# delldu/TransMVSNet

Measured on AMD Instinct MI355X. Metric: depth maps/sec @ DTU 864x1152 N=5 (48/32/8 hyp); Abs depth L1 vs ref, higher is better.
Workload: dtype f32; 1 GPU; DTU 864x1152, N=5 views, cascade 48/32/8, B=1, hot path from FeatureNet outputs (FMT+pathway+stage glue+cost volume+CostRegNet+softmax/WTA); global_batch=1, parallelism=replica1, launch=hip_graph replay

## Files before the change

include/transmvs.h:

```cpp
#ifndef TRANSMVS_H_
#define TRANSMVS_H_

#include <stddef.h>

#ifdef __cplusplus
extern "C" {
#endif

#define TMVS_ABI_VERSION 11

#define TMVS_OK 0
#define TMVS_ERR_ARG (-1)
#define TMVS_ERR_SHAPE (-2)
#define TMVS_ERR_HIP (-3)

#define TMVS_MAX_VIEWS 16

int tmvs_abi_version(void);
const char* tmvs_status_string(int status);

int tmvs_bn_fold(const float* gamma, const float* beta, const float* mean, const float* var, int n, float eps,
                 float* alpha, float* shift);

int tmvs_stage_hypotheses(const float* depth_values, int n_values, const float* prev_depth, int prev_h, int prev_w,
                          int batch, int ndepth, float ratio, int full_h, int full_w, int stage_scale,
                          float* hyp_out, void* stream);

#define TMVS_WARP_PARTIAL 1
#define TMVS_WARP_ROT_PLAIN 2
#define TMVS_WARP_BWD_PLANES 4
#define TMVS_PW_NPARAMS 201
int tmvs_warp_corr(const float* ref_fea, const float* src_fea, const float* proj, const float* hyp,
                   const float* view_w_in, int vw_shift, int vw_offset, int vw_total, const float* pw_params,
                   int batch, int n_src, int channels, int ndepth, int height, int width, int flags,
                   float* sim_out, float* wsum_out, float* view_w_out, void* stream);

int tmvs_aggregate_finalize(float* sim_sum, const float* w_sum, int batch, int ndepth, int height, int width,
                            void* stream);

int tmvs_homo_warping(const float* src_fea, const float* proj, const float* hyp, int batch, int channels,
                      int ndepth, int height, int width, int flags, float* out, void* stream);

typedef struct {
  const float* w[11];
  const float* alpha[10];
  const float* shift[10];
  int base_ch;
} TmvsCostRegWeights;

size_t tmvs_costregnet_workspace(int batch, int depth, int height, int width, int base_ch);
int tmvs_costregnet(const float* x, int batch, int depth, int height, int width, const TmvsCostRegWeights* w,
                    void* workspace, size_t workspace_bytes, float* logits, void* stream);
int tmvs_costregnet_wta(const float* x, const float* hyp, int batch, int depth, int height, int width,
                        const TmvsCostRegWeights* w, void* workspace, size_t workspace_bytes, float clamp_lo,
                        float clamp_hi, float* prob, float* depth_out, float* depth_raw, float* conf, void* stream);

int tmvs_conv3d_bn_relu(const float* x, int batch, int cin, int d, int h, int w, const float* wpk, const float* alpha,
                        const float* shift, int cout, int stride, float* y, void* stream);
int tmvs_deconv3d_bn_relu_add(const float* x, int batch, int cin, int d, int h, int w, const float* wpk,
                              const float* alpha, const float* shift, int cout, const float* skip, float* y,
                              void* stream);

int tmvs_softmax_wta(const float* logits, const float* hyp, int batch, int ndepth, int height, int width,
                     float clamp_lo, float clamp_hi, float* prob, float* depth, float* depth_raw, float* conf,
                     void* stream);

#define TMVS_ENC_WQ 0
#define TMVS_ENC_BQ 1024
#define TMVS_ENC_WK 1056
#define TMVS_ENC_BK 2080
#define TMVS_ENC_WV 2112
#define TMVS_ENC_BV 3136
#define TMVS_ENC_WO 3168
#define TMVS_ENC_BO 4192
#define TMVS_ENC_W1 4224
#define TMVS_ENC_B1 6272
#define TMVS_ENC_W2T 6336
#define TMVS_ENC_B2 8384
#define TMVS_ENC_LN1G 8416
#define TMVS_ENC_LN1B 8448
#define TMVS_ENC_LN2G 8480
#define TMVS_ENC_LN2B 8512
#define TMVS_ENC_NPARAMS 8544
#define TMVS_KV_NFLOATS 160

int tmvs_fmt_embed(const float* feat, long feat_view_stride, const float* pe, int pe_h, int pe_w, int nv,
                   int channels, int height, int width, float* tokens, void* stream);
size_t tmvs_fmt_kv_workspace(int nv, int s_tokens);
int tmvs_fmt_kv(const float* source, int nv, int s_tokens, const float* enc_w, void* workspace,
                size_t workspace_bytes, float* kv, void* stream);
size_t tmvs_fmt_kv_grouped_workspace(int nv, int group_nv, int s_tokens);
int tmvs_fmt_kv_grouped(const float* source, int nv, int group_nv, int s_tokens, const float* enc_w, void* workspace,
                        size_t workspace_bytes, float* kv, void* stream);
int tmvs_fmt_apply(float* x, int nv, int l_tokens, const float* kv, long kv_view_stride, const float* enc_w,
                   void* stream);
int tmvs_fmt_apply_tiled(float* x, int nv, int l_tokens, const float* kv, long kv_view_stride, const float* enc_w,
                         int tiles_per_wave, void* stream);

int tmvs_fmt_pathway(const float* coarse, const float* lateral, long lat_view_stride, const float* w_reduce,
                     const float* w_smooth, int nv, int cc, int cf, int h, int w, float* out, void* stream);

size_t tmvs_fmt_forward_workspace(int nv, int l_tokens);
int tmvs_fmt_forward(const float* stage1, long view_stride, const float* pe, int pe_h, int pe_w, int nv, int height,
                     int width, const float* const* enc_w, void* workspace, size_t workspace_bytes, float* tokens,
                     void* stream);
size_t tmvs_fmt_forward_split_workspace(int nv, int l_tokens);
int tmvs_fmt_forward_split(const float* stage1, long view_stride, const float* pe, int pe_h, int pe_w, int nv,
                           int height, int width, const float* const* enc_w, void* workspace, size_t workspace_bytes,
                           float* tokens, void* stream, void* side_stream);

size_t tmvs_depth_stage_workspace(int ndepth, int height, int width, int base_ch);
int tmvs_depth_stage(const float* depth_values, int n_values, const float* prev_depth, int prev_h, int prev_w,
                     const float* feat, int n_views, int channels, int ndepth, float ratio, int full_h, int full_w,
                     int stage_scale, const float* proj, const float* pw_params, float* view_w, int vw_shift,
                     int warp_flags, const TmvsCostRegWeights* cr, void* workspace, size_t workspace_bytes, float clamp_lo,
                     float clamp_hi, float* hyp_out, float* prob_out, float* depth_out, float* depth_raw_out,
                     float* conf_out, void* stream);

#define TMVS_CONV_TRANSPOSED 1
#define TMVS_CONV_ACCUMULATE 2
int tmvs_conv3d_generic(const float* x, int batch, int cin, int d_in, int h_in, int w_in, const float* w, int cout,
                        int d_out, int h_out, int w_out, int stride, int flags, float* y, void* stream);

int tmvs_conv3d_mfma(const float* x, int batch, int cin, int d, int h, int w, const float* wpk, int cout, int stride,
                     int transposed, const float* skip, float* y, void* stream);

size_t tmvs_conv3d_wgrad_workspace(int batch, int d, int h, int w, int a_ch, int b_ch);
int tmvs_conv3d_wgrad(const float* direct, int a_ch, int batch, int pd, int ph, int pw, const float* gathered,
                      int b_ch, int gd, int gh, int gw, int stride, void* workspace, size_t workspace_bytes,
                      float* dw, void* stream);

size_t tmvs_warp_corr_backward_workspace(int n_src, int channels, int height, int width, int ndepth);
int tmvs_warp_corr_backward(const float* ref_fea, const float* src_fea, const float* proj, const float* hyp,
                            const float* dsim, int n_src, int channels, int ndepth, int height, int width, int flags,
                            void* workspace, size_t workspace_bytes, float* dref, float* dsrc, void* stream);

size_t tmvs_pixelwise_train_workspace(void);
int tmvs_pixelwise_train_forward(const float* sims, int n_views, int ndepth, int height, int width, const float* pwp,
                                 void* workspace, size_t workspace_bytes, float* stats, float* view_w, int* dstar,
                                 void* stream);
int tmvs_aggregate_train(const float* sims, const float* view_w, int n_views, int ndepth, int height, int width,
                         int vw_shift, float* sim, float* wsum, void* stream);
int tmvs_aggregate_train_backward(const float* dsim, const float* sims, const float* sim, const float* wsum,
                                  const float* view_w, int n_views, int ndepth, int height, int width, int vw_shift,
// ... 167 lines not shown
```

transmvsnet_amd/_lib.py:

```python
from __future__ import annotations

import ctypes
import os

_HERE = os.path.dirname(os.path.abspath(__file__))
LIB_PATH = os.environ.get("TMVS_LIB_PATH") or os.path.join(_HERE, "libtransmvs_hip.so")

P = ctypes.c_void_p
I = ctypes.c_int
L = ctypes.c_long
F = ctypes.c_float
S = ctypes.c_size_t
D = ctypes.c_double

SIGNATURES = {
    "tmvs_abi_version": (I, []),
    "tmvs_status_string": (ctypes.c_char_p, [I]),
    "tmvs_bn_fold": (I, [P, P, P, P, I, F, P, P]),
    "tmvs_stage_hypotheses": (I, [P, I, P, I, I, I, I, F, I, I, I, P, P]),
    "tmvs_warp_corr": (I, [P, P, P, P, P, I, I, I, P, I, I, I, I, I, I, I, P, P, P, P]),
    "tmvs_aggregate_finalize": (I, [P, P, I, I, I, I, P]),
    "tmvs_homo_warping": (I, [P, P, P, I, I, I, I, I, I, P, P]),
    "tmvs_costregnet_workspace": (S, [I, I, I, I, I]),
    "tmvs_costregnet": (I, [P, I, I, I, I, P, P, S, P, P]),
    "tmvs_costregnet_wta": (I, [P, P, I, I, I, I, P, P, S, F, F, P, P, P, P, P]),
    "tmvs_conv3d_bn_relu": (I, [P, I, I, I, I, I, P, P, P, I, I, P, P]),
    "tmvs_deconv3d_bn_relu_add": (I, [P, I, I, I, I, I, P, P, P, I, P, P, P]),
    "tmvs_softmax_wta": (I, [P, P, I, I, I, I, F, F, P, P, P, P, P]),
    "tmvs_fmt_embed": (I, [P, L, P, I, I, I, I, I, I, P, P]),
    "tmvs_fmt_kv_workspace": (S, [I, I]),
    "tmvs_fmt_kv": (I, [P, I, I, P, P, S, P, P]),
    "tmvs_fmt_apply": (I, [P, I, I, P, L, P, P]),
    "tmvs_fmt_apply_tiled": (I, [P, I, I, P, L, P, I, P]),
    "tmvs_fmt_pathway": (I, [P, P, L, P, P, I, I, I, I, I, P, P]),
    "tmvs_fmt_forward_workspace": (S, [I, I]),
    "tmvs_fmt_forward": (I, [P, L, P, I, I, I, I, I, P, P, S, P, P]),
    "tmvs_fmt_forward_split_workspace": (S, [I, I]),
    "tmvs_fmt_forward_split": (I, [P, L, P, I, I, I, I, I, P, P, S, P, P, P]),
    "tmvs_fmt_kv_grouped_workspace": (S, [I, I, I]),
    "tmvs_fmt_kv_grouped": (I, [P, I, I, I, P, P, S, P, P]),
    "tmvs_depth_stage_workspace": (S, [I, I, I, I]),
    "tmvs_depth_stage": (I, [P, I, P, I, I, P, I, I, I, F, I, I, I, P, P, P, I, I, P, P, S, F, F, P, P, P, P, P, P]),
    "tmvs_deform_conv2d_packed_floats": (S, [I]),
    "tmvs_deform_conv2d_pack": (I, [P, I, I, P]),
    "tmvs_deform_conv2d": (I, [P, P, P, P, P, P, I, I, I, I, I, I, P, P, P]),
    "tmvs_dcn_fused": (I, [P, P, P, P, P, P, P, I, I, I, I, I, I, P, P, P]),
    "tmvs_conv3x3_nhwc": (I, [P, P, P, P, P, I, I, I, I, I, I, P, P, P]),
    "tmvs_conv3x3_nhwc_acc": (I, [P, P, I, I, I, I, I, P, P]),
    "tmvs_fpn_merge": (I, [P, P, I, P, P, I, I, I, P, P]),
    "tmvs_conv2d_packed_floats": (S, [I, I, I]),
    "tmvs_conv2d_pack": (I, [P, I, I, I, P]),
    "tmvs_conv2d_bn_relu": (I, [P, I, I, I, I, P, I, I, I, P, P, I, P, P]),
    "tmvs_fusibile": (I, [P, P, I, I, I, I, I, F, P, P, P]),
    "tmvs_dynamic_fusion": (I, [P, I, I, I, I, P, I, P, P, P, F, I, I, P, P, P, P, P]),
    "tmvs_depth_postprocess": (I, [P, P, P, P, P, I, I, F, F, F, P, P, P, P, P]),
    "tmvs_resize_bilinear_u8": (I, [P, I, I, P, P, P, P, P, P, I, I, P, P]),
    "tmvs_resize_bilinear_f32": (I, [P, I, I, I, P, P, P, P, P, P, I, I, P, P]),
    "tmvs_entropy_loss_workspace": (S, [I, I, I]),
    "tmvs_entropy_loss": (I, [P, P, I, P, P, I, I, I, I, F, P, S, P, P, P, P, P]),
    "tmvs_depth_metrics_workspace": (S, [I]),
    "tmvs_depth_metrics": (I, [P, P, P, I, F, P, S, P, P]),
    "tmvs_warp_corr_backward_workspace": (S, [I, I, I, I, I]),
    "tmvs_warp_corr_backward": (I, [P, P, P, P, P, I, I, I, I, I, I, P, S, P, P, P]),
    "tmvs_pixelwise_train_workspace": (S, []),
    "tmvs_pixelwise_train_forward": (I, [P, I, I, I, I, P, P, S, P, P, P, P]),
    "tmvs_aggregate_train": (I, [P, P, I, I, I, I, I, P, P, P]),
    "tmvs_aggregate_train_backward": (I, [P, P, P, P, P, I, I, I, I, I, P, P, P]),
    "tmvs_pixelwise_train_backward": (I, [P, I, I, I, I, P, P, P, P, P, P, S, P, P, P]),
    "tmvs_upsample2_add_nhwc": (I, [P, P, I, I, I, I, P, P]),
    "tmvs_upsample2_backward_nhwc": (I, [P, I, I, I, I, P, P]),
    "tmvs_token_linear": (I, [P, L, I, I, P, P, I, P, I, P, P]),
    "tmvs_token_linear_res": (I, [P, L, I, I, P, P, I, P, P, P, P]),
    "tmvs_token_wgrad_workspace": (S, [L, I, I]),
    "tmvs_token_wgrad": (I, [P, I, P, I, L, P, S, P, P, I, P]),
    "tmvs_layer_norm_fwd": (I, [P, L, P, P, P, P]),
    "tmvs_layer_norm_bwd_workspace": (S, [L]),
    "tmvs_layer_norm_bwd": (I, [P, P, L, P, P, S, P, P, I, P]),
    "tmvs_linattn_fwd": (I, [P, L, L, P, L, P, P]),
    "tmvs_linattn_bwd_workspace": (S, [L, L]),
    "tmvs_linattn_bwd_q": (I, [P, P, L, L, P, L, P, S, P, P, P]),
    "tmvs_linattn_bwd_kv": (I, [P, P, L, L, P, P, P, P]),
    "tmvs_adam_step": (I, [P, P, P, P, L, D, D, D, D, D, I, P]),
    "tmvs_adam_step_dev": (I, [P, P, P, P, L, D, P, D, D, D, D, P, P, P]),
    "tmvs_conv3d_generic": (I, [P, I, I, I, I, I, P, I, I, I, I, I, I, P, P]),
    "tmvs_conv3d_mfma": (I, [P, I, I, I, I, I, P, I, I, I, P, P, P]),
    "tmvs_conv3d_wgrad_workspace": (S, [I, I, I, I, I, I]),
    "tmvs_conv3d_wgrad": (I, [P, I, I, I, I, I, P, I, I, I, I, I, P, S, P, P]),
    "tmvs_bn_train_workspace": (S, [L, I]),
    "tmvs_bn_stats": (I, [P, L, I, P, S, P, P, P]),
    "tmvs_bn_relu_train": (I, [P, L, I, P, P, P, P, F, P, P, P]),
    "tmvs_bn_relu_backward": (I, [P, P, L, I, P, P, P, P, F, P, S, P, P, P, P]),
    "tmvs_bn_train_workspace_grouped": (S, [I, L, I]),
    "tmvs_bn_stats_grouped": (I, [P, I, L, I, P, S, P, P, P]),
    "tmvs_bn_relu_train_grouped": (I, [P, I, L, I, P, P, P, P, F, P, P, P]),
    "tmvs_bn_relu_backward_grouped": (I, [P, P, I, L, I, P, P, P, P, F, P, S, P, P, P, P]),
    "tmvs_conv2d_generic": (I, [P, I, I, I, I, P, P, I, I, I, I, I, I, I, P, P]),
    "tmvs_conv2d_wgrad_workspace": (S, [I, I, I, I, I, I]),
    "tmvs_conv2d_wgrad": (I, [P, I, I, I, I, P, I, I, I, I, I, I, P, S, P, P]),
    "tmvs_colsum_workspace": (S, [L, I]),
    "tmvs_colsum": (I, [P, L, I, P, S, P, P]),
    "tmvs_dcn_forward_train": (I, [P, P, P, P, P, I, I, I, I, I, P, P, P, P]),
    "tmvs_dcn_backward_workspace": (S, [I, I, I, I]),
    "tmvs_dcn_backward": (I, [P, P, P, P, I, I, I, I, I, P, S, P, P, P, P]),
    "tmvs_dcn_backward_set": (I, [P, P, P, P, I, I, I, I, I, P, S, P, P, P, P, P]),
    "tmvs_nearest_up2_backward_nhwc": (I, [P, I, I, I, I, I, P, P]),
    "tmvs_softmax_backward": (I, [P, P, I, I, I, I, P, P]),
    "tmvs_dtu_cell_keys": (I, [P, L, P, P, P]),
    "tmvs_dtu_gather_points": (I, [P, P, P, L, P, P]),
    "tmvs_dtu_grid_table_bytes": (S, [L]),
    "tmvs_dtu_grid_table": (I, [P, P, L, L, P, S, P]),
# ... 52 lines not shown
```

transmvsnet_amd/csrc/costreg.hip:

```cpp
#include "common.h"

namespace tmvs {

typedef float floatx4 __attribute__((ext_vector_type(4)));

template <int N>
struct VecN;
template <>
struct VecN<4> {
  float v[4];
  __device__ __forceinline__ void load(const float* p) {
    const float4 t = *reinterpret_cast<const float4*>(p);
    v[0] = t.x;
    v[1] = t.y;
    v[2] = t.z;
    v[3] = t.w;
  }
  __device__ __forceinline__ void zero() { v[0] = v[1] = v[2] = v[3] = 0.f; }
};
template <>
struct VecN<2> {
  float v[2];
  __device__ __forceinline__ void load(const float* p) {
    const float2 t = *reinterpret_cast<const float2*>(p);
    v[0] = t.x;
    v[1] = t.y;
  }
  __device__ __forceinline__ void zero() { v[0] = v[1] = 0.f; }
};

struct Buf {
  __amdgpu_buffer_rsrc_t r;
  __device__ __forceinline__ Buf(const float* base, uint32_t nbytes)
      : r(__builtin_amdgcn_make_buffer_rsrc(const_cast<float*>(base), (short)0, (int)nbytes, 0x00020000)) {}
  static constexpr int kOOB = (int)0x80000000u;
  __device__ __forceinline__ float4 ld4(int voff, int soff = 0) const {
    const auto v = __builtin_amdgcn_raw_buffer_load_b128(r, voff, soff, 0);
    return make_float4(__uint_as_float(v[0]), __uint_as_float(v[1]), __uint_as_float(v[2]), __uint_as_float(v[3]));
  }
  __device__ __forceinline__ float2 ld2(int voff, int soff = 0) const {
    const auto v = __builtin_amdgcn_raw_buffer_load_b64(r, voff, soff, 0);
    return make_float2(__uint_as_float(v[0]), __uint_as_float(v[1]));
  }
};
template <int N>
__device__ __forceinline__ void buf_load(VecN<N>& d, const Buf& b, int voff, int soff = 0);
template <>
__device__ __forceinline__ void buf_load<4>(VecN<4>& d, const Buf& b, int voff, int soff) {
  const float4 t = b.ld4(voff, soff);
  d.v[0] = t.x, d.v[1] = t.y, d.v[2] = t.z, d.v[3] = t.w;
}
template <>
__device__ __forceinline__ void buf_load<2>(VecN<2>& d, const Buf& b, int voff, int soff) {
  const float2 t = b.ld2(voff, soff);
  d.v[0] = t.x, d.v[1] = t.y;
}

struct Geo {
  int Di, Hi, Wi;
  int Do, Ho, Wo;
  float lo;
};

__device__ __forceinline__ float act(float v, float lo) { return v > lo ? v : lo; }

constexpr int kLdsWavesPerEu = 3;
template <int CIN, int COUT, int S, int TD, int TH, int MBB, int WS = 1, bool KDSKIP = false, bool TAPOUT = false>
__global__ __launch_bounds__(256) __attribute__((amdgpu_waves_per_eu(kLdsWavesPerEu, kLdsWavesPerEu))) void conv3d_lds_kernel(const float* __restrict__ x, const float* __restrict__ wpk,
                                                         const float* __restrict__ alpha,
                                                         const float* __restrict__ shift, float* __restrict__ y,
                                                         Geo g) {
  constexpr int CK = CIN < 16 ? CIN : 16;
  constexpr int PL = CK / 4;
  constexpr int MB = (COUT + 15) / 16;
  constexpr int MG = MB / MBB;
  static_assert(WS == 1 || WS == 2 || WS == 4, "WS");
  static_assert(MBB % WS == 0 && (TD * TH * WS) % 4 == 0, "wave split");
  constexpr int NBW = TD * TH * WS / 4, MBW = MBB / WS;
  constexpr int LW = 15 * S + 3, LH = (TH - 1) * S + 3, LD = (TD - 1) * S + 3;
  constexpr bool SWZ = (CK == 16);
  constexpr int VST = SWZ ? 16 : CK + 4;
  constexpr int NVOX = LD * LH * LW;
  static_assert(MB % MBB == 0, "tile");
  static_assert(!TAPOUT || (TD == 1 && !KDSKIP), "TAPOUT: one output slice per workgroup, its own kd skip");
  __shared__ __attribute__((aligned(16))) float tile[(TAPOUT ? CIN / CK : 1) * NVOX * VST];

  const int nws = (g.Wo + 15) / 16, nhs = (g.Ho + TH - 1) / TH, nds = (g.Do + TD - 1) / TD;
  int t = xcd_remap(blockIdx.x, gridDim.x);
  const int mg = t % MG;
  t /= MG;
  const int ws = t % nws;
  t /= nws;
  const int hs = t % nhs;
  t /= nhs;
  const int ds = t % nds;
  const int n = t / nds;
  const int ow0 = ws * 16, oh0 = hs * TH, od0 = ds * TD;
  const int iw0 = ow0 * S - 1, ih0 = oh0 * S - 1, id0 = od0 * S - 1;
  const int lane = threadIdx.x & 63, wv = threadIdx.x >> 6;
  const int col = lane & 15, kgrp = lane >> 4;
  const int rg = __builtin_amdgcn_readfirstlane(wv / WS), bg = __builtin_amdgcn_readfirstlane(wv % WS);
  const int mb0 = mg * MBB + bg * MBW;
  const size_t in_n = (size_t)n * g.Di * g.Hi * g.Wi;

  floatx4 acc[NBW][MBW];
#pragma unroll
  for (int r = 0; r < NBW; ++r)
#pragma unroll
    for (int m = 0; m < MBW; ++m) acc[r][m] = floatx4{0.f, 0.f, 0.f, 0.f};

  constexpr int NCH = CIN / CK, NLD = (NVOX * PL + 255) / 256;
  const Buf xb(x + in_n * CIN, (uint32_t)g.Di * g.Hi * g.Wi * CIN * 4);
  const Buf wb(wpk, 27u * COUT * CIN * 4);
  float4 pf[NLD];
  auto fetch_to = [&](int ch, float4(&dst)[NLD]) {
#pragma unroll
    for (int k = 0; k < NLD; ++k) {
      const int idx = threadIdx.x + 256 * k;
      const int vox = idx / PL, q = idx - vox * PL;
      const int lw = vox % LW, rest = vox / LW, lh = rest % LH, ld = rest / LH;
      const int iw = iw0 + lw, ih = ih0 + lh, id = id0 + ld;
// ... 954 lines not shown
    bool ok[NBW];
#pragma unroll
    for (int r = 0; r < NBW; ++r) {
      const int rr = wv * NBW + r;
      const int md = c.md0 + rr / THI, mh = c.mh0 + rr % THI;
      ok[r] = md < g.Di && mh < g.Hi && ow < 2 * g.Wi;
      oo[r] = (out_n + ((size_t)(2 * md) * g.Ho + 2 * mh) * g.Wo + ow) * 8 + (lane & 1) * 4;
#pragma unroll
      for (int pdh = 0; pdh < 4; ++pdh)
        sk[r][pdh] = (ok[r] && skip) ? *reinterpret_cast<const float4*>(skip + oo[r] + (pdh >> 1) * plane + (pdh & 1) * row)
                           : make_float4(0.f, 0.f, 0.f, 0.f);
    }
    floatx4 acc[NBW][4];
#pragma unroll
    for (int r = 0; r < NBW; ++r)
#pragma unroll
      for (int q = 0; q < 4; ++q) acc[r][q] = floatx4{0.f, 0.f, 0.f, 0.f};
#pragma unroll
    for (int pdh = 0; pdh < 4; ++pdh) {
      const int pd = pdh >> 1, ph = pdh & 1;
#pragma unroll
      for (int td = 0; td < 1 + pd; ++td)
#pragma unroll
        for (int th = 0; th < 1 + ph; ++th) {
          const int kd = pd ? (td ? 2 : 0) : 1, od_off = (pd && !td) ? 1 : 0;
          const int kh = ph ? (th ? 2 : 0) : 1, oh_off = (ph && !th) ? 1 : 0;
          const int tap_base = kd * 9 + kh * 3;
          VecN<PL> a1, a2;
          wfrag(tap_base + (hi ? 2 : 1), a1);
          if (hi)
            wfrag(tap_base + 0, a2);
          else
            a2.zero();
#pragma unroll
          for (int r = 0; r < NBW; ++r) {
            const int rr = wv * NBW + r;
            const int mdl = rr / THI, mhl = rr - mdl * THI;
            const int lv = ((mdl + od_off) * LH + mhl + oh_off) * LW + col;
            VecN<PL> b1, b2;
            b1.load(cur + lv * VST + 4 * (kgrp ^ ((lv >> 1) & 3)));
            b2.load(cur + (lv + 1) * VST + 4 * (kgrp ^ (((lv + 1) >> 1) & 3)));
#pragma unroll
            for (int j = 0; j < PL; ++j)
              acc[r][pdh] = __builtin_amdgcn_mfma_f32_16x16x4f32(a1.v[j], b1.v[j], acc[r][pdh], 0, 0, 0);
#pragma unroll
            for (int j = 0; j < PL; ++j)
              acc[r][pdh] = __builtin_amdgcn_mfma_f32_16x16x4f32(a2.v[j], b2.v[j], acc[r][pdh], 0, 0, 0);
          }
          __builtin_amdgcn_sched_barrier(0);
        }
    }
#pragma unroll
    for (int r = 0; r < NBW; ++r)
#pragma unroll
      for (int pdh = 0; pdh < 4; ++pdh) {
        const floatx4 a = acc[r][pdh];
        *reinterpret_cast<float4*>(eb + (2 * col + (kgrp >> 1)) * 8 + cq) =
            make_float4(act(fmaf(a[0], al.x, sh.x), g.lo), act(fmaf(a[1], al.y, sh.y), g.lo), act(fmaf(a[2], al.z, sh.z), g.lo),
                        act(fmaf(a[3], al.w, sh.w), g.lo));
        __builtin_amdgcn_wave_barrier();
        const float4 v = *reinterpret_cast<const float4*>(eb + lane * 4);
        __builtin_amdgcn_wave_barrier();
        const float4 sv = sk[r][pdh];
        if (ok[r])
          *reinterpret_cast<float4*>(y + oo[r] + (pdh >> 1) * plane + (pdh & 1) * row) =
              make_float4(sv.x + v.x, sv.y + v.y, sv.z + v.z, sv.w + v.w);
      }
    if (tn < t_hi) commit(tile[(it + 1) & 1]);
    __syncthreads();
  }
}

template <int TDI, int THI>
static int launch_deconv_c8(const float* x, const float* w, const float* al, const float* sh, const float* skip,
                            float* y, int B, const Geo& g, hipStream_t st) {
  const long ntiles = (long)B * ((g.Di + TDI - 1) / TDI) * ((g.Hi + THI - 1) / THI) * ((g.Wi + 15) / 16);
  const long grid = persistent_grid(deconv3d_c8_kernel<TDI, THI>, ntiles);
  hipLaunchKernelGGL((deconv3d_c8_kernel<TDI, THI>), dim3((unsigned)grid), dim3(256), 0, st, x, w, al, sh, skip, y, g,
                     (int)ntiles);
  TMVS_CHECK_LAUNCH();
  return TMVS_OK;
}

template <int CIN, int COUT, int TDI, int THI, int MBB>
static int launch_deconv(const float* x, const float* w, const float* al, const float* sh, const float* skip,
                         float* y, int B, const Geo& g, hipStream_t st) {
  constexpr int MG = ((COUT + 15) / 16) / MBB;
  const long nblk = (long)B * ((g.Di + TDI - 1) / TDI) * ((g.Hi + THI - 1) / THI) * ((g.Wi + 15) / 16) * MG;
  hipLaunchKernelGGL((deconv3d_lds_kernel<CIN, COUT, TDI, THI, MBB>), dim3((unsigned)nblk), dim3(256), 0, st, x, w,
                     al, sh, skip, y, g);
  TMVS_CHECK_LAUNCH();
  return TMVS_OK;
}

static int conv_dispatch(const float* x, int B, int cin, int d, int h, int w, const float* wpk, const float* al,
                         const float* sh, int cout, int stride, float* y, hipStream_t st, float lo = 0.f) {
  Geo g;
  g.lo = lo;
  g.Di = d;
  g.Hi = h;
  g.Wi = w;
  if (stride == 1) {
    g.Do = d;
    g.Ho = h;
    g.Wo = w;
  } else {
    g.Do = (d - 1) / 2 + 1;
    g.Ho = (h - 1) / 2 + 1;
    g.Wo = (w - 1) / 2 + 1;
  }
  if ((long long)d * h * w * cin * 4 >= (1LL << 31)) return TMVS_ERR_SHAPE;
  constexpr int kKdSkipMaxDo = 2;
  const bool kdskip = g.Do <= kKdSkipMaxDo;
  constexpr bool KD = true, TAPOUT = true;
  using Conv3Tile = LdsTile<2, 2, 2, 2>;
  using Conv4Tile = LdsTile<2, 2, 2, 2>;
  using Conv4TileKd = LdsTile<2, 4, 2, 1>;
  using Conv5Tile = LdsTile<1, 2, 4, 4>;
  using Conv6Tile = LdsTile<1, 2, 4, 4>;
  int (*launch)(const float*, const float*, const float*, const float*, float*, int, const Geo&, hipStream_t) = nullptr;
  if (stride == 1) {
    if (cin == 16 && cout == 16)
      launch = launch_conv_c16<2, 4>;
    else if (cin == 32 && cout == 32)
      launch = kdskip ? launch_conv<32, 32, 1, Conv4TileKd, KD> : launch_conv<32, 32, 1, Conv4Tile>;
    else if (cin == 64 && cout == 64)
      launch = kdskip ? launch_conv<64, 64, 1, Conv6Tile, KD> : launch_conv<64, 64, 1, Conv6Tile>;
  } else {
    if (cin == 8 && cout == 16)
      launch = launch_conv_s2c8_tile<2, 2>;
    else if (cin == 16 && cout == 32)
      launch = kdskip ? launch_conv<16, 32, 2, Conv3Tile, KD> : launch_conv<16, 32, 2, Conv3Tile>;
    else if (cin == 32 && cout == 64)
      launch = launch_conv<32, 64, 2, Conv5Tile, false, TAPOUT>;
  }
  return launch ? launch(x, wpk, al, sh, y, B, g, st) : TMVS_ERR_SHAPE;
}

static int deconv_dispatch(const float* x, int B, int cin, int d, int h, int w, const float* wpk, const float* al,
                           const float* sh, int cout, const float* skip, float* y, hipStream_t st, float lo = 0.f) {
  Geo g;
  g.lo = lo;
  g.Di = d;
  g.Hi = h;
  g.Wi = w;
  g.Do = 2 * d;
  g.Ho = 2 * h;
  g.Wo = 2 * w;
  const bool even = g.Di % 2 == 0;
  int (*launch)(const float*, const float*, const float*, const float*, const float*, float*, int, const Geo&,
                hipStream_t) = nullptr;
  if (cin == 64 && cout == 32)
    launch = even ? launch_deconv<64, 32, 2, 2, 1> : launch_deconv<64, 32, 1, 4, 1>;
  else if (cin == 32 && cout == 16)
    launch = even ? launch_deconv<32, 16, 2, 2, 1> : launch_deconv<32, 16, 1, 4, 1>;
  else if (cin == 16 && cout == 8)
    launch = even ? launch_deconv_c8<2, 2> : launch_deconv_c8<1, 4>;
  return launch ? launch(x, wpk, al, sh, skip, y, B, g, st) : TMVS_ERR_SHAPE;
}


}

using namespace tmvs;

extern "C" int tmvs_conv3d_bn_relu(const float* x, int batch, int cin, int d, int h, int w, const float* wpk,
                                   const float* alpha, const float* shift, int cout, int stride, float* y,
                                   void* stream) {
  if (!x || !wpk || !alpha || !shift || !y || batch <= 0 || d <= 0 || h <= 0 || w <= 0) return TMVS_ERR_ARG;
  if (stride != 1 && stride != 2) return TMVS_ERR_ARG;
  return conv_dispatch(x, batch, cin, d, h, w, wpk, alpha, shift, cout, stride, y, (hipStream_t)stream);
}

extern "C" int tmvs_deconv3d_bn_relu_add(const float* x, int batch, int cin, int d, int h, int w, const float* wpk,
                                         const float* alpha, const float* shift, int cout, const float* skip,
                                         float* y, void* stream) {
  if (!x || !wpk || !alpha || !shift || !skip || !y || batch <= 0 || d <= 0 || h <= 0 || w <= 0)
    return TMVS_ERR_ARG;
  return deconv_dispatch(x, batch, cin, d, h, w, wpk, alpha, shift, cout, skip, y, (hipStream_t)stream);
}

static int launch_prob(const float* x, float* y, int batch, int D, int H, int W, const float* wt, hipStream_t st) {
  constexpr int NR = 1;
  const dim3 grid((unsigned)(((W + kProbCols - 1) / kProbCols) * ((H + 4 * NR - 1) / (4 * NR)) * batch *
                             ((D + kDChunk - 1) / kDChunk)));
  hipLaunchKernelGGL(prob_kernel<NR>, grid, dim3(256), 0, st, x, y, D, H, W, wt);
  TMVS_CHECK_LAUNCH();
  return TMVS_OK;
}

__device__ float kUnitAlpha[64] = {1.f, 1.f, 1.f, 1.f, 1.f, 1.f, 1.f, 1.f, 1.f, 1.f, 1.f, 1.f, 1.f, 1.f, 1.f, 1.f,
                                   1.f, 1.f, 1.f, 1.f, 1.f, 1.f, 1.f, 1.f, 1.f, 1.f, 1.f, 1.f, 1.f, 1.f, 1.f, 1.f,
                                   1.f, 1.f, 1.f, 1.f, 1.f, 1.f, 1.f, 1.f, 1.f, 1.f, 1.f, 1.f, 1.f, 1.f, 1.f, 1.f,
                                   1.f, 1.f, 1.f, 1.f, 1.f, 1.f, 1.f, 1.f, 1.f, 1.f, 1.f, 1.f, 1.f, 1.f, 1.f, 1.f};
__device__ float kZeroShift[64];

extern "C" int tmvs_conv3d_mfma(const float* x, int batch, int cin, int d, int h, int w, const float* wpk, int cout,
                                int stride, int transposed, const float* skip, float* y, void* stream) {
  if (!x || !wpk || !y || batch <= 0 || d <= 0 || h <= 0 || w <= 0) return TMVS_ERR_ARG;
  if (transposed ? stride != 2 : (stride != 1 && stride != 2)) return TMVS_ERR_ARG;
  if (skip && !transposed) return TMVS_ERR_ARG;
  int dev = 0;
  if (hipGetDevice(&dev) != hipSuccess || dev < 0 || dev >= 64) return TMVS_ERR_HIP;
  static const float* unit[64][2];
  if (!unit[dev][0]) {
    void *a, *b;
    if (hipGetSymbolAddress(&a, HIP_SYMBOL(kUnitAlpha)) != hipSuccess ||
        hipGetSymbolAddress(&b, HIP_SYMBOL(kZeroShift)) != hipSuccess)
      return TMVS_ERR_HIP;
    unit[dev][1] = (const float*)b;
    unit[dev][0] = (const float*)a;
  }
  const float *al = unit[dev][0], *sh = unit[dev][1];
  const float lo = -__builtin_huge_valf();
  hipStream_t st = (hipStream_t)stream;
  if (!transposed && stride == 1 && cin == 1 && cout == 8) {
    if ((long long)d * h * w * 32 >= (1LL << 31)) return TMVS_ERR_SHAPE;
    const dim3 grid((unsigned)(((w + kProbCols - 1) / kProbCols) * ((h + 3) / 4) * batch * ((d + kDChunk - 1) / kDChunk)));
    hipLaunchKernelGGL(conv0_kernel, grid, dim3(256), 0, st, x, y, d, h, w, wpk, al, sh, lo);
    TMVS_CHECK_LAUNCH();
    return TMVS_OK;
  }
  if (!transposed && stride == 1 && cin == 8 && cout == 1) {
    if ((long long)d * h * w * 32 >= (1LL << 31)) return TMVS_ERR_SHAPE;
    return launch_prob(x, y, batch, d, h, w, wpk, st);
  }
  if (transposed) return deconv_dispatch(x, batch, cin, d, h, w, wpk, al, sh, cout, skip, y, st, lo);
  return conv_dispatch(x, batch, cin, d, h, w, wpk, al, sh, cout, stride, y, st, lo);
}

static size_t align_up(size_t v) { return (v + 255) & ~(size_t)255; }

extern "C" size_t tmvs_costregnet_workspace(int batch, int depth, int height, int width, int base_ch) {
  const size_t v0 = (size_t)batch * depth * height * width;
  const size_t v1 = v0 / 8, v2 = v0 / 64, v3 = v0 / 512;
  const size_t c = (size_t)base_ch;
  size_t bytes = 0;
  bytes += align_up(v0 * c * 4);
  bytes += align_up(v1 * 2 * c * 4) * 2;
  bytes += align_up(v2 * 4 * c * 4) * 2;
  bytes += align_up(v3 * 8 * c * 4) * 2;
  bytes += align_up(v2 * 4 * c * 4);
  bytes += align_up(v1 * 2 * c * 4);
  bytes += align_up(v0 * c * 4);
  return bytes;
}

static int costregnet_trunk(const float* x, int batch, int depth, int height, int width, const TmvsCostRegWeights* w,
                            void* workspace, size_t workspace_bytes, hipStream_t st, float** x11_out,
                            float** c0_out) {
  if (!x || !w || !workspace || batch <= 0) return TMVS_ERR_ARG;
  if (depth % 8 || height % 8 || width % 8) return TMVS_ERR_SHAPE;
  if (w->base_ch != 8) return TMVS_ERR_SHAPE;
  if ((long long)depth * height * width * 32 >= (1LL << 31)) return TMVS_ERR_SHAPE;
  for (int i = 0; i < 11; ++i)
    if (!w->w[i]) return TMVS_ERR_ARG;
  for (int i = 0; i < 10; ++i)
    if (!w->alpha[i] || !w->shift[i]) return TMVS_ERR_ARG;
  if (workspace_bytes < tmvs_costregnet_workspace(batch, depth, height, width, w->base_ch)) return TMVS_ERR_ARG;
  const int c = w->base_ch;
  const size_t v0 = (size_t)batch * depth * height * width;
  const size_t v1 = v0 / 8, v2 = v0 / 64, v3 = v0 / 512;
// ... 93 lines not shown
```

transmvsnet_amd/ops.py:

```python
from __future__ import annotations

import ctypes

import numpy as np
import torch

from . import _lib

_lib_h = _lib.load


_TIMER = None


def set_timer(timer):
    global _TIMER
    _TIMER = timer


class _Span:
    __slots__ = ("tok",)

    def __init__(self, name):
        self.tok = _TIMER.begin(name) if _TIMER is not None else None
# ... 185 lines not shown


def costregnet(x, weights: "_lib.CostRegWeights", keepalive=None):
    _dev(x, "x")
    b, d, h, w = x.shape
    nbytes = _lib_h().tmvs_costregnet_workspace(b, d, h, w, weights.base_ch)
    ws = torch.empty(nbytes // 4 + 64, device=x.device)
    out = torch.empty_like(x)
    with _Span("tmvs_costregnet"):
        _lib.check(_lib_h().tmvs_costregnet(_ptr(x), b, d, h, w, ctypes.byref(weights), _ptr(ws), ws.numel() * 4,
                                            _ptr(out), _stream()), "tmvs_costregnet")
    return out


def costregnet_wta(x, weights: "_lib.CostRegWeights", hyp, clamp=(425.0, 935.0)):
    _dev(x, "x")
    _dev(hyp, "hyp")
    b, d, h, w = x.shape
    if tuple(hyp.shape) != (b, d, h, w):
        raise ValueError(f"costregnet_wta: hyp shape {tuple(hyp.shape)} != volume shape {(b, d, h, w)}")
    nbytes = _lib_h().tmvs_costregnet_workspace(b, d, h, w, weights.base_ch)
    ws = torch.empty(nbytes // 4 + 64, device=x.device)
    prob = torch.empty_like(x)
    depth = torch.empty(b, h, w, device=x.device)
    raw = torch.empty_like(depth)
    conf = torch.empty_like(depth)
    with _Span("tmvs_costregnet"):
        _lib.check(_lib_h().tmvs_costregnet_wta(_ptr(x), _ptr(hyp), b, d, h, w, ctypes.byref(weights), _ptr(ws),
                                                ws.numel() * 4, ctypes.c_float(clamp[0]), ctypes.c_float(clamp[1]),
                                                _ptr(prob), _ptr(depth), _ptr(raw), _ptr(conf), _stream()),
                   "tmvs_costregnet_wta")
    return prob, depth, raw, conf


def _layer_args(op, x, wpk, alpha, shift, cout):
    if x.dim() != 5:
        raise ValueError(f"{op}: x must be NDHWC [B, D, H, W, cin]")
    for name, t in (("x", x), ("wpk", wpk), ("alpha", alpha), ("shift", shift)):
        _layer_tensor(op, name, t, x.device)
    cin = x.shape[4]
    if wpk.numel() != 27 * cout * cin:
        raise ValueError(f"{op}: wpk must hold 27 * cout * cin = {27 * cout * cin} floats, not {wpk.numel()}")
    for name, t in (("alpha", alpha), ("shift", shift)):
        if t is not None and t.numel() < cout:
            raise ValueError(f"{op}: {name} must hold cout = {cout} floats, not {t.numel()}")


def _layer_tensor(op, name, t, device):
    if t is None:
        return
    if not t.is_cuda or t.device != device:
        raise ValueError(f"{op}: {name} must be a GPU tensor on x's device (the HIP path has no CPU fallback)")
    if t.dtype != torch.float32 or not t.is_contiguous():
        raise ValueError(f"{op}: {name} must be contiguous float32")


def _layer_like(op, name, t, shape, device):
    _layer_tensor(op, name, t, device)
    if t is not None and tuple(t.shape) != tuple(shape):
        raise ValueError(f"{op}: {name} must be a contiguous {list(shape)} tensor, not {list(t.shape)}")


def _layer_no_alias(op, skip, out):
    if skip is not None and out is not None and skip.data_ptr() == out.data_ptr():
        raise ValueError(f"{op}: out must not alias skip (the kernels read skip while they write out)")


def _conv_out_dhw(d, h, w, stride):
    return (d, h, w) if stride == 1 else ((d - 1) // 2 + 1, (h - 1) // 2 + 1, (w - 1) // 2 + 1)


def conv3d_bn_relu(x, wpk, alpha, shift, cout, stride, out=None):
    _layer_args("conv3d_bn_relu", x, wpk, alpha, shift, cout)
    b, d, h, w, cin = x.shape
    shape = (b, *_conv_out_dhw(d, h, w, stride), cout)
    _layer_like("conv3d_bn_relu", "out", out, shape, x.device)
    y = torch.empty(shape, device=x.device) if out is None else out
    with _Span("tmvs_conv3d_bn_relu"):
        _lib.check(_lib_h().tmvs_conv3d_bn_relu(_ptr(x), b, cin, d, h, w, _ptr(wpk), _ptr(alpha), _ptr(shift), cout,
                                                stride, _ptr(y), _stream()), "tmvs_conv3d_bn_relu")
    return y


def deconv3d_bn_relu_add(x, wpk, alpha, shift, cout, skip, out=None):
    _layer_args("deconv3d_bn_relu_add", x, wpk, alpha, shift, cout)
    b, d, h, w, cin = x.shape
    shape = (b, 2 * d, 2 * h, 2 * w, cout)
    if skip is None:
        raise ValueError("deconv3d_bn_relu_add: skip is required")
    _layer_like("deconv3d_bn_relu_add", "skip", skip, shape, x.device)
    _layer_like("deconv3d_bn_relu_add", "out", out, shape, x.device)
    _layer_no_alias("deconv3d_bn_relu_add", skip, out)
    y = torch.empty(shape, device=x.device) if out is None else out
    with _Span("tmvs_deconv3d_bn_relu_add"):
        _lib.check(_lib_h().tmvs_deconv3d_bn_relu_add(_ptr(x), b, cin, d, h, w, _ptr(wpk), _ptr(alpha), _ptr(shift),
                                                      cout, _ptr(skip), _ptr(y), _stream()), "tmvs_deconv3d_bn_relu_add")
    return y


def fmt_embed(feat_nchw, pe, out_tokens):
    nv, c, h, w = feat_nchw.shape
    with _Span("tmvs_fmt_embed"):
        _lib.check(_lib_h().tmvs_fmt_embed(_ptr(feat_nchw), c * h * w, _ptr(pe), pe.shape[1], pe.shape[2], nv, c, h, w,
                                           _ptr(out_tokens), _stream()), "tmvs_fmt_embed")
    return out_tokens


def fmt_kv(source_tokens, enc_w, out=None, group_nv=None):
    nv, s, _ = source_tokens.shape
    group_nv = nv if group_nv is None else int(group_nv)
    nbytes = _lib_h().tmvs_fmt_kv_grouped_workspace(nv, group_nv, s)
    ws = torch.empty(max(1, nbytes // 4), device=source_tokens.device)
    kv = out if out is not None else torch.empty(nv, _lib.KV_NFLOATS, device=source_tokens.device)
    with _Span("tmvs_fmt_kv"):
        _lib.check(_lib_h().tmvs_fmt_kv_grouped(_ptr(source_tokens), nv, group_nv, s, _ptr(enc_w), _ptr(ws),
                                                ws.numel() * 4, _ptr(kv), _stream()), "tmvs_fmt_kv_grouped")
    return kv


def fmt_apply(x_tokens, kv, enc_w, shared_kv=False, tiles_per_wave=0):
    nv, l, _ = x_tokens.shape
    with _Span("tmvs_fmt_apply"):
        _lib.check(_lib_h().tmvs_fmt_apply_tiled(_ptr(x_tokens), nv, l, _ptr(kv), 0 if shared_kv else _lib.KV_NFLOATS,
                                                 _ptr(enc_w), int(tiles_per_wave), _stream()), "tmvs_fmt_apply")
    return x_tokens


def fmt_pathway(coarse_nhwc, lateral_nchw, w_reduce, w_smooth, out=None):
    nv, h, w, cc = coarse_nhwc.shape
    cf = lateral_nchw.shape[1]
    if out is None:
        out = torch.empty(nv, 2 * h, 2 * w, cf, device=coarse_nhwc.device)
    elif tuple(out.shape) != (nv, 2 * h, 2 * w, cf) or not out.is_contiguous():
        raise ValueError(f"fmt_pathway: out must be a contiguous [{nv},{2 * h},{2 * w},{cf}] tensor")
    with _Span("tmvs_fmt_pathway"):
        _lib.check(_lib_h().tmvs_fmt_pathway(_ptr(coarse_nhwc), _ptr(lateral_nchw), cf * 4 * h * w, _ptr(w_reduce),
                                             _ptr(w_smooth), nv, cc, cf, h, w, _ptr(out), _stream()), "tmvs_fmt_pathway")
    return out


def fmt_forward(stage1_nchw, pe, enc_list, tokens=None, side_stream=None):
    _dev(stage1_nchw, "stage1")
    nv, c, h, w = stage1_nchw.shape
    tokens = torch.empty(nv, h * w, c, device=stage1_nchw.device) if tokens is None else tokens
    split = side_stream is not None and nv > 1
    lib = _lib_h()
    nbytes = lib.tmvs_fmt_forward_split_workspace(nv, h * w) if split else lib.tmvs_fmt_forward_workspace(nv, h * w)
    ws = torch.empty(nbytes // 4 + 64, device=stage1_nchw.device)
    ptrs = (ctypes.c_void_p * 8)(*[e.data_ptr() for e in enc_list])
    args = (_ptr(stage1_nchw), c * h * w, _ptr(pe), pe.shape[1], pe.shape[2], nv, h, w, ptrs, _ptr(ws), ws.numel() * 4,
            _ptr(tokens), _stream())
    with _Span("tmvs_fmt_forward"):
        if split:
            _lib.check(lib.tmvs_fmt_forward_split(*args, side_stream.cuda_stream), "tmvs_fmt_forward_split")
            if not torch.cuda.is_current_stream_capturing():
                ws.record_stream(side_stream)
                tokens.record_stream(side_stream)
        else:
            _lib.check(lib.tmvs_fmt_forward(*args), "tmvs_fmt_forward")
    return tokens


def depth_stage(depth_values, prev_depth, feat_nhwc, ndepth, ratio, full_hw, stage_scale, proj12, pw_params,
                view_w, vw_shift, cr_weights, clamp=(425.0, 935.0), rot_order="auto"):
    _dev(depth_values, "depth_values")
    _dev(prev_depth, "prev_depth")
    _dev(feat_nhwc, "feat")
    _dev(view_w, "view_w")
    n, h, w, c = feat_nhwc.shape
    dev = feat_nhwc.device
    hyp = torch.empty(1, ndepth, h, w, device=dev)
    prob = torch.empty_like(hyp)
    depth = torch.empty(1, h, w, device=dev)
    raw = torch.empty_like(depth)
    conf = torch.empty_like(depth)
    nbytes = _lib_h().tmvs_depth_stage_workspace(ndepth, h, w, cr_weights.base_ch)
    ws = torch.empty(nbytes // 4 + 64, device=dev)
    proj = np.ascontiguousarray(proj12, np.float32).reshape(n - 1, 12)
    pw = None if pw_params is None else np.ascontiguousarray(pw_params, np.float32)
# ... 881 lines not shown
```

Before: 302.3 depth_maps/s.

## Add persistent software-pipelined MFMA kernel for 32→16 transposed 3D conv

```diff
diff --git a/include/transmvs.h b/include/transmvs.h
--- a/include/transmvs.h
+++ b/include/transmvs.h
@@ -60,6 +60,12 @@
 int tmvs_deconv3d_bn_relu_add(const float* x, int batch, int cin, int d, int h, int w, const float* wpk,
                               const float* alpha, const float* shift, int cout, const float* skip, float* y,
                               void* stream);
+int tmvs_deconv3d_bn_relu_add_generic(const float* x, int batch, int cin, int d, int h, int w, const float* wpk,
+                                      const float* alpha, const float* shift, int cout, const float* skip, float* y,
+                                      void* stream);
+int tmvs_deconv3d_bn_relu_add_persistent(const float* x, int batch, int cin, int d, int h, int w, const float* wpk,
+                                         const float* alpha, const float* shift, int cout, const float* skip,
+                                         float* y, int max_workgroups, void* stream);
 
 int tmvs_softmax_wta(const float* logits, const float* hyp, int batch, int ndepth, int height, int width,
                      float clamp_lo, float clamp_hi, float* prob, float* depth, float* depth_raw, float* conf,
diff --git a/transmvsnet_amd/_lib.py b/transmvsnet_amd/_lib.py
--- a/transmvsnet_amd/_lib.py
+++ b/transmvsnet_amd/_lib.py
@@ -26,6 +26,8 @@
     "tmvs_costregnet_wta": (I, [P, P, I, I, I, I, P, P, S, F, F, P, P, P, P, P]),
     "tmvs_conv3d_bn_relu": (I, [P, I, I, I, I, I, P, P, P, I, I, P, P]),
     "tmvs_deconv3d_bn_relu_add": (I, [P, I, I, I, I, I, P, P, P, I, P, P, P]),
+    "tmvs_deconv3d_bn_relu_add_generic": (I, [P, I, I, I, I, I, P, P, P, I, P, P, P]),
+    "tmvs_deconv3d_bn_relu_add_persistent": (I, [P, I, I, I, I, I, P, P, P, I, P, P, I, P]),
     "tmvs_softmax_wta": (I, [P, P, I, I, I, I, F, F, P, P, P, P, P]),
     "tmvs_fmt_embed": (I, [P, L, P, I, I, I, I, I, I, P, P]),
     "tmvs_fmt_kv_workspace": (S, [I, I]),
diff --git a/transmvsnet_amd/csrc/costreg.hip b/transmvsnet_amd/csrc/costreg.hip
--- a/transmvsnet_amd/csrc/costreg.hip
+++ b/transmvsnet_amd/csrc/costreg.hip
@@ -1,4 +1,6 @@
 #include "common.h"
+
+#include <utility>
 
 namespace tmvs {
 
@@ -37,6 +39,11 @@
   __device__ __forceinline__ float4 ld4(int voff, int soff = 0) const {
     const auto v = __builtin_amdgcn_raw_buffer_load_b128(r, voff, soff, 0);
     return make_float4(__uint_as_float(v[0]), __uint_as_float(v[1]), __uint_as_float(v[2]), __uint_as_float(v[3]));
+  }
+  __device__ __forceinline__ void st4(float4 v, int voff) const {
+    typedef unsigned uintx4 __attribute__((ext_vector_type(4)));
+    const uintx4 u{__float_as_uint(v.x), __float_as_uint(v.y), __float_as_uint(v.z), __float_as_uint(v.w)};
+    __builtin_amdgcn_raw_buffer_store_b128(u, r, voff, 0, 0);
   }
   __device__ __forceinline__ float2 ld2(int voff, int soff = 0) const {
     const auto v = __builtin_amdgcn_raw_buffer_load_b64(r, voff, soff, 0);
@@ -1157,6 +1164,222 @@
   return TMVS_OK;
 }
 
+struct DeconvTap {
+  int cls, tap, off;
+};
+constexpr DeconvTap deconv_stream_tap(int stream, int i) {
+  int k = 0;
+  for (int cls = 0; cls < 8; ++cls) {
+    if ((cls == 0 || cls == 3 || cls == 7) != (stream == 0)) continue;
+    const int pd = cls >> 2, ph = (cls >> 1) & 1, pw = cls & 1;
+    for (int td = 0; td < 1 + pd; ++td)
+      for (int th = 0; th < 1 + ph; ++th)
+        for (int tw = 0; tw < 1 + pw; ++tw) {
+          const int kd = pd ? (td ? 2 : 0) : 1, od_off = (pd && !td) ? 1 : 0;
+          const int kh = ph ? (th ? 2 : 0) : 1, oh_off = (ph && !th) ? 1 : 0;
+          const int kw = pw ? (tw ? 2 : 0) : 1, ow_off = (pw && !tw) ? 1 : 0;
+          if (k++ == i) return DeconvTap{cls, kd * 9 + kh * 3 + kw, od_off * 4 + oh_off * 2 + ow_off};
+        }
+  }
+  return DeconvTap{-1, 0, 0};
+}
+constexpr int deconv_class_done(int i) {
+  for (int st = 0; st < 2; ++st) {
+    const DeconvTap t = deconv_stream_tap(st, i);
+    if (t.cls >= 0 && deconv_stream_tap(st, i + 1).cls != t.cls) return t.cls;
+  }
+  return -1;
+}
+static_assert(deconv_stream_tap(0, 12).cls == 7 && deconv_stream_tap(0, 13).cls < 0, "stream 0: 13 taps");
+static_assert(deconv_stream_tap(1, 13).cls == 6 && deconv_stream_tap(1, 14).cls < 0, "stream 1: 14 taps");
+
+template <typename F, int... I>
+__device__ __forceinline__ void static_for(std::integer_sequence<int, I...>, F f) {
+  (f(std::integral_constant<int, I>{}), ...);
+}
+
+template <int TDI, int THI>
+__global__ __launch_bounds__(256) __attribute__((amdgpu_waves_per_eu(2, 2))) void deconv3d_c16p_kernel(
+    const float* __restrict__ x, const float* __restrict__ wpk, const float* __restrict__ alpha,
+    const float* __restrict__ shift, const float* __restrict__ skip, float* __restrict__ y, Geo g, int ntiles) {
+  constexpr int CIN = 32, COUT = 16, PL = 4, NCH = 2;
+  static_assert(TDI * THI == 4, "one input-grid row per wave");
+  constexpr int LW = 17, LH = THI + 1, LD = TDI + 1, VST = 16;
+  constexpr int NVOX = LD * LH * LW;
+  constexpr int NQ = NVOX * 2 * PL;
+  constexpr int NLD = (NQ + 255) / 256;
+  __shared__ __attribute__((aligned(16))) float tile[NCH][NVOX * VST];
+  __shared__ __attribute__((aligned(16))) float wts[NCH][27 * 16 * 16];
+
+  const int nws = (g.Wi + 15) / 16, nhs = (g.Hi + THI - 1) / THI, nds = (g.Di + TDI - 1) / TDI;
+  const int lane = threadIdx.x & 63, wv = __builtin_amdgcn_readfirstlane(threadIdx.x >> 6);
+  const int col = lane & 15, kgrp = lane >> 4;
+  const int nxcd = gridDim.x >= 8 ? 8 : 1, per_xcd = gridDim.x / nxcd;
+  const int xcd = blockIdx.x % nxcd, kx = blockIdx.x / nxcd;
+  const int t_lo = (int)((long)ntiles * xcd / nxcd), t_hi = (int)((long)ntiles * (xcd + 1) / nxcd);
+  if (kx >= per_xcd) return;
+
+  struct TileCoord {
+    int n, md0, mh0, mw0;
+  };
+  auto coord = [&](int t) {
+    TileCoord c;
+    c.mw0 = (t % nws) * 16;
+    t /= nws;
+    c.mh0 = (t % nhs) * THI;
+    t /= nhs;
+    c.md0 = (t % nds) * TDI;
+    c.n = t / nds;
+    return c;
+  };
+  const uint32_t in_bytes = (uint32_t)g.Di * g.Hi * g.Wi * CIN * 4;
+  const uint32_t out_bytes = (uint32_t)g.Do * g.Ho * g.Wo * COUT * 4;
+  float4 pf[NLD];
+  struct Fetch {
+    Buf xb;
+    TileCoord c;
+    int soff;
+    bool live;
+  };
+  auto fetch_of = [&](int t, bool live) {
+    const TileCoord c = coord(live ? t : 0);
+    return Fetch{Buf(x + (size_t)c.n * g.Di * g.Hi * g.Wi * CIN, in_bytes), c,
+                 ((c.md0 * g.Hi + c.mh0) * g.Wi + c.mw0) * CIN * 4 , live};
+  };
+  auto fetch1 = [&](const Fetch& f, int k) {
+    const int idx = threadIdx.x + 256 * k;
+    const int vox = idx >> 3, q8 = idx & 7;
+    const int lw = vox % LW, rest = vox / LW, lh = rest % LH, ld = rest / LH;
+    const bool ok = f.live && idx < NQ && f.c.mw0 + lw < g.Wi && f.c.mh0 + lh < g.Hi && f.c.md0 + ld < g.Di;
+    pf[k] = f.xb.ld4(ok ? (((ld * g.Hi + lh) * g.Wi + lw) * CIN + 4 * q8) * 4 : Buf::kOOB, f.soff);
+  };
+  auto fetch = [&](int t, bool live) {
+    const Fetch f = fetch_of(t, live);
+#pragma unroll
+    for (int k = 0; k < NLD; ++k) fetch1(f, k);
+  };
+  auto commit = [&]() {
+#pragma unroll
+    for (int k = 0; k < NLD; ++k) {
+      const int idx = threadIdx.x + 256 * k;
+      const int vox = idx >> 3, q8 = idx & 7;
+      const int ch = q8 >> 2, q = q8 & 3;
+      if (idx < NQ) *reinterpret_cast<float4*>(tile[ch] + vox * VST + 4 * (q ^ ((vox >> 1) & 3))) = pf[k];
+    }
+  };
+
+  constexpr int NWQ = NCH * 27 * 16 * 4, NWL = (NWQ + 255) / 256;
+  const Buf wb(wpk, 27u * COUT * CIN * 4);
+  float4 wreg[NWL];
+#pragma unroll
+  for (int k = 0; k < NWL; ++k) {
+    const int idx = threadIdx.x + 256 * k;
+    wreg[k] = wb.ld4(idx < NWQ ? idx * 16 : Buf::kOOB);
+  }
+  int t = t_lo + kx;
+  fetch(t, t < t_hi);
+#pragma unroll
+  for (int k = 0; k < NWL; ++k) {
+    const int idx = threadIdx.x + 256 * k;
+    const int q = idx & 3, ch = (idx >> 2) & 1, row = (idx >> 3) & 15, tap = idx >> 7;
+    if (idx < NWQ) *reinterpret_cast<float4*>(wts[ch] + (tap * 16 + row) * 16 + 4 * (q ^ ((row >> 1) & 3))) = wreg[k];
+  }
+  const int co = kgrp * 4;
+  const float4 al = *reinterpret_cast<const float4*>(alpha + co);
+  const float4 sh = *reinterpret_cast<const float4*>(shift + co);
+  const int mdl = wv / THI, mhl = wv - mdl * THI;
+  const int woff = col * 16 + 4 * (kgrp ^ ((col >> 1) & 3));
+
+  commit();
+  __syncthreads();
+  for (; t < t_hi; t += per_xcd) {
+    const TileCoord c = coord(t);
+    const int tn = t + per_xcd;
+    const bool more = tn < t_hi;
+    const Fetch fn = fetch_of(tn, more);
+    const int md = c.md0 + mdl, mh = c.mh0 + mhl, mw = c.mw0 + col;
+    const bool ok = md < g.Di && mh < g.Hi && mw < g.Wi;
+    const size_t out_n = (size_t)c.n * g.Do * g.Ho * g.Wo * COUT;
+    const Buf sb(skip ? skip + out_n : nullptr, skip ? out_bytes : 0u), yb(y + out_n, out_bytes);
+    const int o0 = (((2 * md) * g.Ho + 2 * mh) * g.Wo + 2 * mw) * COUT + co;
+    int so[8];
+    float4 sk[8];
+#pragma unroll
+    for (int cls = 0; cls < 8; ++cls) {
+      const int rel = (((cls >> 2) * g.Ho + ((cls >> 1) & 1)) * g.Wo + (cls & 1)) * COUT;
+      so[cls] = ok ? (o0 + rel) * 4 : Buf::kOOB;
+    }
+    floatx4 acc[8];
+#pragma unroll
+    for (int cls = 0; cls < 8; ++cls) acc[cls] = floatx4{0.f, 0.f, 0.f, 0.f};
+    auto epilogue = [&](auto cc) {
+      constexpr int cls = decltype(cc)::value;
+      const float4 s = sk[cls];
+      float4 v;
+      v.x = s.x + act(fmaf(acc[cls][0], al.x, sh.x), g.lo);
+      v.y = s.y + act(fmaf(acc[cls][1], al.y, sh.y), g.lo);
+      v.z = s.z + act(fmaf(acc[cls][2], al.z, sh.z), g.lo);
+      v.w = s.w + act(fmaf(acc[cls][3], al.w, sh.w), g.lo);
+      yb.st4(v, so[cls]);
+    };
+    VecN<PL> b[NCH][8], a[2][2];
+    auto bload = [&](int ch, int off) {
+      const int lvox = ((mdl + (off >> 2)) * LH + mhl + ((off >> 1) & 1)) * LW + col + (off & 1);
+      b[ch][off].load(tile[ch] + lvox * VST + 4 * (kgrp ^ ((lvox >> 1) & 3)));
+    };
+#pragma unroll
+    for (int off = 0; off < 8; ++off) bload(0, off);
+    a[0][0].load(wts[0] + deconv_stream_tap(0, 0).tap * 256 + woff);
+    a[0][1].load(wts[0] + deconv_stream_tap(1, 0).tap * 256 + woff);
+    __builtin_amdgcn_sched_barrier(0);
+    static_for(std::make_integer_sequence<int, 14 * NCH>{}, [&](auto sc) {
+      constexpr int s = decltype(sc)::value, ch = s / 14, i = s % 14;
+      constexpr DeconvTap t0 = deconv_stream_tap(0, i), t1 = deconv_stream_tap(1, i);
+      constexpr int s1 = s + 1, ch1 = s1 / 14, i1 = s1 % 14;
+      constexpr bool next = s1 < 14 * NCH, next0 = next && deconv_stream_tap(0, i1).cls >= 0;
+      if constexpr (next0) a[s1 & 1][0].load(wts[ch1] + deconv_stream_tap(0, i1).tap * 256 + woff);
+      if constexpr (next) a[s1 & 1][1].load(wts[ch1] + deconv_stream_tap(1, i1).tap * 256 + woff);
+      if constexpr (s < 8) bload(1, s);
+      if constexpr (s < 8) sk[s] = sb.ld4(so[s]);
+      if constexpr (s >= 8 && s < 8 + NLD) fetch1(fn, s - 8);
+#pragma unroll
+      for (int j = 0; j < PL; ++j) {
+        if constexpr (t0.cls >= 0)
+          acc[t0.cls] = __builtin_amdgcn_mfma_f32_16x16x4f32(a[s & 1][0].v[j], b[ch][t0.off].v[j], acc[t0.cls], 0, 0, 0);
+        acc[t1.cls] = __builtin_amdgcn_mfma_f32_16x16x4f32(a[s & 1][1].v[j], b[ch][t1.off].v[j], acc[t1.cls], 0, 0, 0);
+      }
+      __builtin_amdgcn_sched_group_barrier(0x100, (next0 ? 1 : 0) + (next ? 1 : 0) + (s < 8 ? 1 : 0), 0);
+      __builtin_amdgcn_sched_group_barrier(0x008, t0.cls >= 0 ? 2 * PL : PL, 0);
+      if constexpr (ch == NCH - 1 && i >= 1 && deconv_class_done(i - 1) >= 0)
+        epilogue(std::integral_constant<int, deconv_class_done(i - 1)>{});
+      __builtin_amdgcn_sched_barrier(0);
+    });
+    epilogue(std::integral_constant<int, deconv_class_done(13)>{});
+    __syncthreads();
+    commit();
+    __syncthreads();
+  }
+}
+
+template <typename K>
+static int persistent_cap(K kernel) {
+  return persistent_grid(kernel, 1L << 40);
+}
+
+constexpr int kC16pMinTilesNum = 3, kC16pMinTilesDen = 2;
+
+template <int TDI, int THI>
+static int launch_deconv_c16p(const float* x, const float* w, const float* al, const float* sh, const float* skip,
+                              float* y, int B, const Geo& g, hipStream_t st, int max_wgs = 0) {
+  const long ntiles = (long)B * ((g.Di + TDI - 1) / TDI) * ((g.Hi + THI - 1) / THI) * ((g.Wi + 15) / 16);
+  long grid = persistent_grid(deconv3d_c16p_kernel<TDI, THI>, ntiles);
+  if (max_wgs > 0) grid = std::min<long>(grid, max_wgs);
+  hipLaunchKernelGGL((deconv3d_c16p_kernel<TDI, THI>), dim3((unsigned)grid), dim3(256), 0, st, x, w, al, sh, skip, y, g,
+                     (int)ntiles);
+  TMVS_CHECK_LAUNCH();
+  return TMVS_OK;
+}
+
 template <int CIN, int COUT, int TDI, int THI, int MBB>
 static int launch_deconv(const float* x, const float* w, const float* al, const float* sh, const float* skip,
                          float* y, int B, const Geo& g, hipStream_t st) {
@@ -1212,8 +1435,11 @@
   return launch ? launch(x, wpk, al, sh, y, B, g, st) : TMVS_ERR_SHAPE;
 }
 
+enum class Route { kAuto, kGeneric, kPersistent };
+
 static int deconv_dispatch(const float* x, int B, int cin, int d, int h, int w, const float* wpk, const float* al,
-                           const float* sh, int cout, const float* skip, float* y, hipStream_t st, float lo = 0.f) {
+                           const float* sh, int cout, const float* skip, float* y, hipStream_t st, float lo = 0.f,
+                           Route route = Route::kAuto, int max_wgs = 0) {
   Geo g;
   g.lo = lo;
   g.Di = d;
@@ -1231,6 +1457,18 @@
     launch = even ? launch_deconv<32, 16, 2, 2, 1> : launch_deconv<32, 16, 1, 4, 1>;
   else if (cin == 16 && cout == 8)
     launch = even ? launch_deconv_c8<2, 2> : launch_deconv_c8<1, 4>;
+  if (cin == 32 && cout == 16 && route != Route::kGeneric) {
+    const bool fits = (long long)g.Do * g.Ho * g.Wo * cout * 4 < (1LL << 31);
+    const int tdi = even ? 2 : 1, thi = even ? 2 : 4;
+    const long ntiles = (long)B * ((d + tdi - 1) / tdi) * ((h + thi - 1) / thi) * ((w + 15) / 16);
+    const int cap = even ? persistent_cap(deconv3d_c16p_kernel<2, 2>) : persistent_cap(deconv3d_c16p_kernel<1, 4>);
+    if (route == Route::kPersistent && !fits) return TMVS_ERR_SHAPE;
+    if (route == Route::kPersistent || (fits && ntiles * kC16pMinTilesDen >= (long)cap * kC16pMinTilesNum))
+      return even ? launch_deconv_c16p<2, 2>(x, wpk, al, sh, skip, y, B, g, st, max_wgs)
+                  : launch_deconv_c16p<1, 4>(x, wpk, al, sh, skip, y, B, g, st, max_wgs);
+  } else if (route == Route::kPersistent) {
+    return TMVS_ERR_SHAPE;
+  }
   return launch ? launch(x, wpk, al, sh, skip, y, B, g, st) : TMVS_ERR_SHAPE;
 }
 
@@ -1253,6 +1491,25 @@
   if (!x || !wpk || !alpha || !shift || !skip || !y || batch <= 0 || d <= 0 || h <= 0 || w <= 0)
     return TMVS_ERR_ARG;
   return deconv_dispatch(x, batch, cin, d, h, w, wpk, alpha, shift, cout, skip, y, (hipStream_t)stream);
+}
+
+extern "C" int tmvs_deconv3d_bn_relu_add_generic(const float* x, int batch, int cin, int d, int h, int w,
+                                                 const float* wpk, const float* alpha, const float* shift, int cout,
+                                                 const float* skip, float* y, void* stream) {
+  if (!x || !wpk || !alpha || !shift || !skip || !y || batch <= 0 || d <= 0 || h <= 0 || w <= 0)
+    return TMVS_ERR_ARG;
+  return deconv_dispatch(x, batch, cin, d, h, w, wpk, alpha, shift, cout, skip, y, (hipStream_t)stream, 0.f,
+                         Route::kGeneric);
+}
+
+extern "C" int tmvs_deconv3d_bn_relu_add_persistent(const float* x, int batch, int cin, int d, int h, int w,
+                                                    const float* wpk, const float* alpha, const float* shift,
+                                                    int cout, const float* skip, float* y, int max_workgroups,
+                                                    void* stream) {
+  if (!x || !wpk || !alpha || !shift || !skip || !y || batch <= 0 || d <= 0 || h <= 0 || w <= 0 || max_workgroups < 0)
+    return TMVS_ERR_ARG;
+  return deconv_dispatch(x, batch, cin, d, h, w, wpk, alpha, shift, cout, skip, y, (hipStream_t)stream, 0.f,
+                         Route::kPersistent, max_workgroups);
 }
 
 static int launch_prob(const float* x, float* y, int batch, int D, int H, int W, const float* wt, hipStream_t st) {
diff --git a/transmvsnet_amd/ops.py b/transmvsnet_amd/ops.py
--- a/transmvsnet_amd/ops.py
+++ b/transmvsnet_amd/ops.py
@@ -291,7 +291,7 @@
     return y
 
 
-def deconv3d_bn_relu_add(x, wpk, alpha, shift, cout, skip, out=None):
+def deconv3d_bn_relu_add(x, wpk, alpha, shift, cout, skip, out=None, route=None, max_workgroups=0):
     _layer_args("deconv3d_bn_relu_add", x, wpk, alpha, shift, cout)
     b, d, h, w, cin = x.shape
     shape = (b, 2 * d, 2 * h, 2 * w, cout)
@@ -301,9 +301,13 @@
     _layer_like("deconv3d_bn_relu_add", "out", out, shape, x.device)
     _layer_no_alias("deconv3d_bn_relu_add", skip, out)
     y = torch.empty(shape, device=x.device) if out is None else out
-    with _Span("tmvs_deconv3d_bn_relu_add"):
-        _lib.check(_lib_h().tmvs_deconv3d_bn_relu_add(_ptr(x), b, cin, d, h, w, _ptr(wpk), _ptr(alpha), _ptr(shift),
-                                                      cout, _ptr(skip), _ptr(y), _stream()), "tmvs_deconv3d_bn_relu_add")
+    if route not in (None, "generic", "persistent"):
+        raise ValueError(f"deconv3d_bn_relu_add: unknown route {route!r}")
+    name = "tmvs_deconv3d_bn_relu_add" + ("_" + route if route else "")
+    tail = (int(max_workgroups), _stream()) if route == "persistent" else (_stream(),)
+    with _Span(name):
+        _lib.check(getattr(_lib_h(), name)(_ptr(x), b, cin, d, h, w, _ptr(wpk), _ptr(alpha), _ptr(shift), cout,
+                                           _ptr(skip), _ptr(y), *tail), name)
     return y
 
 
```

Result: faster. 305.8 depth_maps/s, median of 6 (+1.1%).
